# sepsamavi/safe-interactive-crowdnav

Hardware: AMD Instinct MI355X
Metric: sampled trajectories/sec (N x K, 50 denoise steps) (higher is better)
Workload: dtype fp16 activations x split-fp16 weights (weight-lo term as one bf8 MFMA per k64), fp32 accumulate; 1 GPU; cfg3: 256 episodes/GPU x N=5 x K=20 x H=12, 50 DDIM steps, JMID; episodes_per_gpu=256, total_episodes=256, humans=5, samples=20, horizon=12, denoise_steps=50, net=jmid, precision=f16mx, class_default_precision=f16mx, lanes=2

## Files before the change

### safe-interactive-crowdnav_amd/csrc/common.hpp

```cpp
#pragma once
#include <hip/hip_runtime.h>
#include <hip/hip_fp16.h>
#include <stdint.h>

#include <atomic>
#include <mutex>

namespace jmid {

typedef float f32x4 __attribute__((ext_vector_type(4)));
typedef float f32x16 __attribute__((ext_vector_type(16)));
typedef _Float16 f16x8 __attribute__((ext_vector_type(8)));
typedef _Float16 f16x4 __attribute__((ext_vector_type(4)));
typedef _Float16 f16x2 __attribute__((ext_vector_type(2)));

constexpr int kWave = 64;
constexpr int kPeMaxLen = 24;

struct HyperLayout {
    int g1, b1, g3, b3, g4, b4, go, bo, total;
};
__host__ __device__ inline HyperLayout make_hyper_layout(int d_model, int d_mid, int d_low) {
    HyperLayout L;
    L.g1 = 0;
// ... 55 lines not shown
    const Words w = __builtin_bit_cast(Words, a);
#pragma unroll
    for (unsigned i = 0; i < sizeof(T) / 4; ++i) asm volatile("" ::"s"(w.w[i]));
}
template <typename... T>
__device__ __forceinline__ void args_now_each(const T&... t) { (args_now(t), ...); }

__device__ __forceinline__ unsigned long long pin_uniform(unsigned long long v) {
    asm volatile("" : "+s"(v));
    return v;
}
__device__ __forceinline__ unsigned long long pin_uniform_rfl(unsigned long long v) {
    const unsigned lo = __builtin_amdgcn_readfirstlane((unsigned)v), hi = __builtin_amdgcn_readfirstlane((unsigned)(v >> 32));
    unsigned long long u = ((unsigned long long)hi << 32) | lo;
    asm volatile("" : "+s"(u));
    return u;
}

struct Tuning {
    int fuse_embed = 1;
    int ln_fuse = 0;
    int ln_rows = 0;
    int bystander_lds = 0;
    int gemm_h_variant = 0;
    int gemm_ng = 0;
    int no_vt_direct = 0;
    int attn_h_variant = 0;
    int attn_pack = 1;
    int vt_stage = 0;
    int graph = 0;
    int attn_nsplit = 0;
    int csl_swap = 0;
    int attn_sm = 0;
    int attn_prio = 0;
    int attn_one_wg = 0;
    int h1_stage = 0;
    int out_traj = 0;
    int attn_mx = 0;
    int mx_ln = 0;
    int attn_pf = 0;
    int gemm_small = 0;
    int small_cmb = 0;
    int small_lnx = 0;
    int cus = 256;
    int lnx_polls = 0;
    int lnx_withhold = 0;
    int small_lnx2 = 0;
    int gemm_pn = 0;
    int small_lanes = 0;
    int small_qk = 0;
    int small_pn = 0;
    int qkv0 = 0;
    int tail_fold = 0;
    int attn_abl = 0;
    int gemm_abl = 0;
};
#ifdef JMID_ABLATIONS
inline int attn_abl_bits(const Tuning& t) { return t.attn_abl; }
inline int gemm_abl_bits(const Tuning& t) { return t.gemm_abl; }
#else
inline int attn_abl_bits(const Tuning&) { return 0; }
inline int gemm_abl_bits(const Tuning&) { return 0; }
#endif

struct DevSeen {
    std::atomic<bool> v[64];
    DevSeen() { for (auto& b : v) b.store(false, std::memory_order_relaxed); }
};
struct DeviceOnce {
    std::unique_lock<std::mutex> lk;
    std::atomic<bool>* slot = nullptr;
    explicit operator bool() const { return slot != nullptr; }
    DeviceOnce() = default;
    DeviceOnce(DeviceOnce&& o) noexcept : lk(std::move(o.lk)), slot(o.slot) { o.slot = nullptr; }
    ~DeviceOnce() { if (slot) slot->store(true, std::memory_order_release); }
};
inline std::mutex& device_once_mutex() {
    static std::mutex m;
    return m;
}
inline DeviceOnce first_use_on_device(DevSeen& seen) {
    int dev = 0;
    (void)hipGetDevice(&dev);
    dev &= 63;
    DeviceOnce o;
    if (seen.v[dev].load(std::memory_order_acquire)) return o;
    o.lk = std::unique_lock<std::mutex>(device_once_mutex());
    if (seen.v[dev].load(std::memory_order_acquire)) {
        o.lk.unlock();
        return o;
    }
    o.slot = &seen.v[dev];
    return o;
}

template <auto Kernel, size_t MaxLds = 0, typename... Args>
inline hipError_t launch_with_lds(dim3 grid, dim3 block, size_t lds_bytes, hipStream_t st, Args... args) {
    static DevSeen seen;
    if (auto once_ = first_use_on_device(seen))
        (void)hipFuncSetAttribute(reinterpret_cast<const void*>(Kernel), hipFuncAttributeMaxDynamicSharedMemorySize,
                                  (int)(MaxLds ? MaxLds : lds_bytes));
    hipLaunchKernelGGL(Kernel, grid, block, lds_bytes, st, args...);
    return hipGetLastError();
}

template <typename F>
// ... 29 lines not shown
```

### safe-interactive-crowdnav_amd/csrc/gemm_f16x3.hpp

```cpp
#pragma once
#include <type_traits>
#include "common.hpp"
#include "gemm_f32.hpp"

namespace jmid {

typedef _Float16 half_t;
constexpr float kWScale = 256.0f;
constexpr float kWInv = 1.0f / 256.0f;
constexpr float kHalfMax = 60000.0f;

__device__ __forceinline__ void split_f32(float v, half_t& hi, half_t& lo) {
    asm("" : "+v"(v));
    hi = (half_t)v;
    lo = (half_t)(v - (float)hi);
}
__device__ __forceinline__ void split_f32_unscaled(float v, half_t& hi, half_t& lo) { split_f32(v, hi, lo); }
__device__ __forceinline__ unsigned char bf8_of_f16(half_t v) {
    return (unsigned char)((__builtin_bit_cast(unsigned short, v) + 0x80u) >> 8);
}

typedef int i32x2_s __attribute__((ext_vector_type(2)));
typedef unsigned short u16x2_s __attribute__((ext_vector_type(2)));
constexpr unsigned kHalfMaxBits = 0x7B53;
// ... 969 lines not shown
            __syncthreads();
            if (vt_staged_store<X2>(g, acc, m0 + wr * 64, n0 + wc * 128, lds + wid * 8192, l31, hi, lane)) return;
        }
    }
    gemm_h_epilogue<WM, WN, EPI, OUT, X2>(g, acc, m0, n0, wr, wc, l31, hi, BM, BN);
}

template <int EPI, int OUT, bool X2 = false>
inline hipError_t launch_gemm_h_dma256x256(const GemmHArgs& g, hipStream_t st, int flags = 3, int abl = 0) {
    const int ntm = (g.M + 255) / 256, ntn = g.N / 256;
    return launch_with_lds<&gemm_f16x3_dma256x256_kernel<EPI, OUT, X2>>(dim3(ntm * ntn), dim3(512), DMA3_LDS_BYTES, st, g, ntm, ntn,
                                                                         (abl & 8) ? 0 : 1, flags);
}

typedef int i32x4 __attribute__((ext_vector_type(4)));
typedef int i32x8 __attribute__((ext_vector_type(8)));

static __global__ void w8_image_kernel(const float* W, unsigned char* out, int N, int K, float scale) {
    const size_t n = (size_t)N * K;
    const int nb32 = N / 32;
    for (size_t i = (size_t)blockIdx.x * blockDim.x + threadIdx.x; i < n; i += (size_t)gridDim.x * blockDim.x) {
        const int r = (int)(i / K), k = (int)(i % K);
        float v = W[i] * scale;
        asm("" : "+v"(v));
        const half_t h = (half_t)v;
        const half_t lo = (half_t)(v - (float)h);
        const int kb = k >> 6, kk = k & 63, ksg = kk >> 4, hh = (kk >> 3) & 1, e = kk & 7;
        const int p = ksg * 8 + e, lane = (r & 31) + 32 * hh;
        const size_t o = ((((size_t)kb * nb32 + (r >> 5)) * 2 + (p >> 4)) * 64 + lane) * 16 + (p & 15);
        out[o] = (unsigned char)((__builtin_bit_cast(unsigned short, lo) + 0x80u) >> 8);
    }
}

__device__ __forceinline__ int bf8_of_f16x4(int d0, int d1) {
    return (int)__builtin_amdgcn_perm((unsigned)(d1 + 0x00800080), (unsigned)(d0 + 0x00800080), 0x07050301u);
}

template <int WR, int WC, int WM, int WN, int NS>
struct MxCfg {
    static constexpr int NT = 64 * WR * WC, BM = 32 * WM * WR, BN = 32 * WN * WC;
    static constexpr int A_HALFS = BM * 32, W_HALFS = BN * 32, STAGE = A_HALFS + W_HALFS;
    static constexpr int W8_BYTES = BN * 64;
    static constexpr int PIECE = NT * 8;
    static constexpr int NA = A_HALFS / PIECE, NW = W_HALFS / PIECE, N8 = W8_BYTES / (NT * 16);
    static constexpr size_t W8_OFF = size_t(NS) * STAGE * sizeof(half_t);
    static constexpr size_t RING_BYTES = W8_OFF + 2 * W8_BYTES;
    static constexpr size_t VT_BYTES = (WM == 2 && WN == 4) ? size_t(WR * WC) * 16384 : 0;
    static constexpr size_t LDS_BYTES = RING_BYTES > VT_BYTES ? RING_BYTES : VT_BYTES;
    static_assert(NA >= 1 && NW >= 1 && N8 >= 1 && A_HALFS % PIECE == 0 && W_HALFS % PIECE == 0, "tile / workgroup mismatch");
};
template <int N>
__device__ __forceinline__ void wait_vmcnt() { asm volatile("s_waitcnt vmcnt(%0)" ::"n"(N) : "memory"); }

template <int EPI, int OUT, int WR, int WC, int WM, int WN, int NS, bool K8IMG = false>
__global__ __launch_bounds__(64 * WR * WC, (WR * WC == 4 && WM == 2 && NS > 2) ? 1 : 2) void gemm_mx_kernel(GemmHArgs g, int ntm, int ntn, int stage_vt) {
    using C = MxCfg<WR, WC, WM, WN, NS>;
    constexpr int BM = C::BM, BN = C::BN, L = NS - 1;
    extern __shared__ __attribute__((aligned(16))) unsigned char lds_raw[];
    half_t* lds = reinterpret_cast<half_t*>(lds_raw);
    const int tid = threadIdx.x, lane = tid & 63, wid = tid >> 6;
    const int l31 = lane & 31, hi = lane >> 5;
    const int wr = wid / WC, wc = wid % WC;
    const int nwg = gridDim.x, b = blockIdx.x;
    const int q8 = nwg / 8, r8 = nwg % 8, xcd = b % 8;
    const int swz = (xcd < r8 ? xcd * (q8 + 1) : r8 * (q8 + 1) + (xcd - r8) * q8) + b / 8;
    const int gw = (stage_vt >> 8) ? (stage_vt >> 8) : ntn;
    const int per_g = ntm * gw, cg = swz / per_g, rem_g = swz - cg * per_g;
    const int tm = rem_g / gw, tn = cg * gw + (rem_g - tm * gw);
    const int m0 = tm * BM, n0 = tn * BN;
    const int nk = g.K / GEMMH_BK;
    const int nrb = (g.M + 127) / 128;
    const half_t* srcA[C::NA];
    const half_t* srcW[C::NW];
#pragma unroll
    for (int p = 0; p < C::NA; ++p) {
        const int h0 = (m0 & 127) * 32 + p * C::PIECE;
        int rb = m0 / 128 + h0 / 4096;
        rb = rb < nrb ? rb : nrb - 1;
        srcA[p] = g.Ahi + (size_t)rb * nk * 4096 + h0 % 4096;
    }
#pragma unroll
    for (int p = 0; p < C::NW; ++p) {
        const int h0 = (n0 & 127) * 32 + p * C::PIECE;
        srcW[p] = g.Whi + (size_t)(n0 / 128 + h0 / 4096) * nk * 4096 + h0 % 4096;
    }
    const unsigned char* src8 = g.W8 + (size_t)(n0 / 32) * 2048;
    unsigned lane_off = (unsigned)tid * 16u;
    const size_t w8_kstride = (size_t)(g.N / 32) * 2048;
    unsigned char* lds8 = lds_raw + C::W8_OFF;
    auto dma16 = [&](const void* s, void* d) {
        const unsigned long long u = pin_uniform(reinterpret_cast<unsigned long long>(s));
        __builtin_amdgcn_global_load_lds(reinterpret_cast<const __attribute__((address_space(1))) char*>(u) + lane_off,
                                         (__attribute__((address_space(3))) void*)d, 16, 0, 0);
    };
    const int wid_s = __builtin_amdgcn_readfirstlane(wid);
    auto issue = [&](int kt, int stg) {
        half_t* st = lds + stg * C::STAGE + wid_s * 512;
#pragma unroll
        for (int p = 0; p < C::NA; ++p) dma16(srcA[p] + (size_t)kt * 4096, st + p * C::PIECE);
#pragma unroll
        for (int p = 0; p < C::NW; ++p) dma16(srcW[p] + (size_t)kt * 4096, st + C::A_HALFS + p * C::PIECE);
        if (kt & 1) {
            const unsigned char* s8 = src8 + (size_t)(kt >> 1) * w8_kstride;
            unsigned char* d8 = lds8 + ((kt >> 1) & 1) * C::W8_BYTES + wid_s * 1024;
#pragma unroll
            for (int q = 0; q < C::N8; ++q) dma16(s8 + q * C::NT * 16, d8 + q * C::NT * 16);
        }
    };
    f32x16 acc[WM][WN];
#pragma unroll
    for (int i = 0; i < WM; ++i)
#pragma unroll
        for (int j = 0; j < WN; ++j)
#pragma unroll
            for (int r = 0; r < 16; ++r) acc[i][j][r] = 0.f;
    int offA[WM][2], offW[WN][2];
#pragma unroll
    for (int i = 0; i < WM; ++i) {
        const int row = wr * WM * 32 + i * 32 + l31, r = row & 127;
#pragma unroll
        for (int ks = 0; ks < 2; ++ks)
            offA[i][ks] = (row >> 7) * DMA_PLANE + r * 32 + (((ks * 2 + hi) ^ ((r >> 2) & 3)) * 8);
    }
#pragma unroll
    for (int j = 0; j < WN; ++j) {
        const int row = wc * WN * 32 + j * 32 + l31, r = row & 127;
#pragma unroll
        for (int ks = 0; ks < 2; ++ks)
            offW[j][ks] = C::A_HALFS + (row >> 7) * DMA_PLANE + r * 32 + (((ks * 2 + hi) ^ ((r >> 2) & 3)) * 8);
    }
    i32x8 a8[WM];
    auto tile = [&](const half_t* st, auto half_c, auto swap_c) {
        constexpr int HALF = decltype(half_c)::value;
        constexpr bool SWAP = decltype(swap_c)::value;
#pragma unroll
        for (int ks = 0; ks < 2; ++ks) {
            f16x8 ah[WM], wh[WN];
#pragma unroll
            for (int i = 0; i < WM; ++i) ah[i] = *reinterpret_cast<const f16x8*>(st + offA[i][ks]);
#pragma unroll
            for (int j = 0; j < WN; ++j) wh[j] = *reinterpret_cast<const f16x8*>(st + offW[j][ks]);
#pragma unroll
            for (int i = 0; i < WM; ++i)
#pragma unroll
                for (int j = 0; j < WN; ++j)
                    acc[i][j] = SWAP ? __builtin_amdgcn_mfma_f32_32x32x16_f16(wh[j], ah[i], acc[i][j], 0, 0, 0)
                                     : __builtin_amdgcn_mfma_f32_32x32x16_f16(ah[i], wh[j], acc[i][j], 0, 0, 0);
#pragma unroll
            for (int i = 0; i < WM; ++i) {
                const i32x4 d = __builtin_bit_cast(i32x4, ah[i]);
                a8[i][HALF * 4 + ks * 2 + 0] = bf8_of_f16x4(d[0], d[1]);
                a8[i][HALF * 4 + ks * 2 + 1] = bf8_of_f16x4(d[2], d[3]);
            }
        }
    };
    auto top = [&](int kt, int stg_next, auto par_c) {
        constexpr int P = decltype(par_c)::value;
        constexpr int n_odd = P == 0 ? L / 2 : (L - 1) / 2;
        if (kt + L - 1 < nk) wait_vmcnt<(L - 1) * (C::NA + C::NW) + n_odd * C::N8>();
        else wait_vmcnt<0>();
        __builtin_amdgcn_s_barrier();
        __builtin_amdgcn_sched_barrier(0);
        asm volatile("" : "+v"(lane_off));
        if (kt + L < nk) issue(kt + L, stg_next);
    };
    auto kloop = [&](auto swap_c) {
        constexpr bool SWAP = decltype(swap_c)::value;
#pragma unroll
        for (int t = 0; t < L; ++t)
            if (t < nk) issue(t, t);
        int stg = 0;
        for (int kt = 0; kt < nk; kt += 2) {
            const int s1 = stg + 1 == NS ? 0 : stg + 1, s2 = s1 + 1 == NS ? 0 : s1 + 1;
            top(kt, stg == 0 ? NS - 1 : stg - 1, std::integral_constant<int, 0>{});
            tile(lds + stg * C::STAGE, std::integral_constant<int, 0>{}, swap_c);
            __builtin_amdgcn_sched_barrier(0);
            top(kt + 1, stg, std::integral_constant<int, 1>{});
            tile(lds + s1 * C::STAGE, std::integral_constant<int, 1>{}, swap_c);
            {
                const unsigned char* wb = lds8 + ((kt >> 1) & 1) * C::W8_BYTES;
                i32x8 w8[WN];
#pragma unroll
                for (int j = 0; j < WN; ++j) {
                    const unsigned char* p = wb + (size_t)((wc * WN + j) * 2) * 1024 + lane * 16;
                    const i32x4 lo = *reinterpret_cast<const i32x4*>(p);
                    const i32x4 up = *reinterpret_cast<const i32x4*>(p + 1024);
                    w8[j] = i32x8{lo[0], lo[1], lo[2], lo[3], up[0], up[1], up[2], up[3]};
                }
#pragma unroll
                for (int i = 0; i < WM; ++i)
#pragma unroll
                    for (int j = 0; j < WN; ++j)
                        acc[i][j] = SWAP ? __builtin_amdgcn_mfma_scale_f32_32x32x64_f8f6f4(w8[j], a8[i], acc[i][j], 1, 1, 0, 0, 0, 0)
                                         : __builtin_amdgcn_mfma_scale_f32_32x32x64_f8f6f4(a8[i], w8[j], acc[i][j], 1, 1, 0, 0, 0, 0);
            }
            __builtin_amdgcn_sched_barrier(0);
            stg = s2;
        }
    };
    if constexpr (OUT == OUT_QKV && WM == 2 && WN == 4) {
        if (((stage_vt & 2) || (K8IMG && g.K8h && (n0 >= g.d || g.Q8l))) && n0 < 2 * g.d && g.d % 128 == 0) {
            kloop(std::true_type{});
            __syncthreads();
            qk_staged_store<K8IMG>(g, acc, m0 + wr * 64, n0 + wc * 128, lds + wid * 8192, l31, hi, lane);
            return;
        }
    }
    if constexpr ((EPI == EPI_CSL && (OUT == OUT_F32 || OUT == OUT_SPLIT)) || (EPI == EPI_BIAS_RELU && OUT == OUT_SPLIT)) {
        if (stage_vt & (EPI == EPI_CSL ? 4 : 8)) {
            kloop(std::true_type{});
            csl_swapped_epilogue<WM, WN, EPI, OUT, true>(g, acc, m0 + wr * WM * 32, n0 + wc * WN * 32, l31, hi);
            return;
        }
    }
    if constexpr (EPI == EPI_BIAS_RELU && OUT == OUT_SPLIT && WM == 2 && WN == 4) {
        if (stage_vt & 16) {
            kloop(std::true_type{});
            __syncthreads();
            h1_staged_store(g, acc, m0 + wr * 64, n0 + wc * 128, lds + wid * 8192, l31, hi, lane);
            return;
        }
    }
    kloop(std::false_type{});
    if constexpr (OUT == OUT_QKV && WM == 2 && WN == 4) {
        if (g.vt_direct && g.hd == 128 && n0 >= 2 * g.d && (stage_vt & 1)) {
            __syncthreads();
            if (vt_staged_store<true>(g, acc, m0 + wr * 64, n0 + wc * 128, lds + wid * 8192, l31, hi, lane)) return;
        }
    }
    gemm_h_epilogue<WM, WN, EPI, OUT, true, OUT == OUT_QKV && !(WM == 2 && WN == 4)>(g, acc, m0, n0, wr, wc, l31, hi, BM, BN);
}

template <int EPI, int OUT, int WR, int WC, int WM, int WN, int NS, bool K8IMG = false>
inline hipError_t launch_gemm_mx_cfg(const GemmHArgs& g, hipStream_t st, int flags, int group_tiles) {
    using C = MxCfg<WR, WC, WM, WN, NS>;
    if constexpr (OUT == OUT_QKV && WM == 2 && WN == 4 && !K8IMG)
        if (g.K8h) return launch_gemm_mx_cfg<EPI, OUT, WR, WC, WM, WN, NS, true>(g, st, flags, group_tiles);
    const int ntm = (g.M + C::BM - 1) / C::BM, ntn = g.N / C::BN;
    return launch_with_lds<&gemm_mx_kernel<EPI, OUT, WR, WC, WM, WN, NS, K8IMG>>(dim3(ntm * ntn), dim3(C::NT), C::LDS_BYTES, st, g, ntm, ntn,
                                                                                  flags | (group_tiles << 8));
}

constexpr int DMA64_PLANE = 64 * 32;
constexpr int DMA64_STAGE = 4 * DMA64_PLANE;
constexpr size_t DMA64_LDS_BYTES = size_t(4) * DMA64_STAGE * sizeof(half_t);

template <int EPI, int OUT, bool X2 = false>
__global__ __launch_bounds__(256, 2) void gemm_f16x3_dma64_kernel(GemmHArgs g, int ntm, int ntn) {
    constexpr int WM = 1, WN = 1, BM = 64, BN = 64;
    extern __shared__ __attribute__((aligned(16))) unsigned char lds_raw[];
    half_t* lds = reinterpret_cast<half_t*>(lds_raw);
    const int tid = threadIdx.x, lane = tid & 63, wid = tid >> 6;
    const int l31 = lane & 31, hi = lane >> 5;
    const int wr = wid >> 1, wc = wid & 1;
    const int nwg = gridDim.x, b = blockIdx.x;
    const int q8 = nwg / 8, r8 = nwg % 8, xcd = b % 8;
    const int swz = (xcd < r8 ? xcd * (q8 + 1) : r8 * (q8 + 1) + (xcd - r8) * q8) + b / 8;
    const int tm = swz / ntn, tn = swz - tm * ntn;
    const int m0 = tm * BM, n0 = tn * BN;
    const int nk = g.K / GEMMH_BK;
    const half_t* src[4];
    src[0] = g.Ahi + ((size_t)(tm >> 1) * nk) * 4096 + (tm & 1) * 2048 + tid * 8;
    src[1] = g.Alo + ((size_t)(tm >> 1) * nk) * 4096 + (tm & 1) * 2048 + tid * 8;
    src[2] = g.Whi + ((size_t)(tn >> 1) * nk) * 4096 + (tn & 1) * 2048 + tid * 8;
    src[3] = g.Wlo + ((size_t)(tn >> 1) * nk) * 4096 + (tn & 1) * 2048 + tid * 8;
    auto issue = [&](int kt) {
        half_t* st = lds + (kt & 3) * DMA64_STAGE + wid * 512;
#pragma unroll
        for (int i = 0; i < 4; ++i)
            __builtin_amdgcn_global_load_lds((const __attribute__((address_space(1))) void*)(src[i] + (size_t)kt * 4096),
                                             (__attribute__((address_space(3))) void*)(st + i * DMA64_PLANE), 16, 0, 0);
    };
    f32x16 accm[1][1];
#pragma unroll
    for (int r = 0; r < 16; ++r) {
        accm[0][0][r] = 0.f;
    }
    const int rowA = wr * 32 + l31, rowW = wc * 32 + l31;
    int offA[2], offW[2];
#pragma unroll
    for (int ks = 0; ks < 2; ++ks) {
        offA[ks] = rowA * 32 + (((ks * 2 + hi) ^ ((rowA >> 2) & 3)) * 8);
        offW[ks] = rowW * 32 + (((ks * 2 + hi) ^ ((rowW >> 2) & 3)) * 8);
    }
    issue(0);
    if (nk > 1) issue(1);
    if (nk > 2) issue(2);
    for (int kt = 0; kt < nk; ++kt) {
        if (kt + 2 < nk) asm volatile("s_waitcnt vmcnt(8)" ::: "memory");
        else if (kt + 1 < nk) asm volatile("s_waitcnt vmcnt(4)" ::: "memory");
        else asm volatile("s_waitcnt vmcnt(0)" ::: "memory");
        __builtin_amdgcn_s_barrier();
        __builtin_amdgcn_sched_barrier(0);
        if (kt + 3 < nk) issue(kt + 3);
        const half_t* st = lds + (kt & 3) * DMA64_STAGE;
#pragma unroll
        for (int ks = 0; ks < 2; ++ks) {
            f16x8 ah[1], al[1], wh[1], wl[1];
            ah[0] = *reinterpret_cast<const f16x8*>(st + offA[ks]);
            al[0] = *reinterpret_cast<const f16x8*>(st + DMA64_PLANE + offA[ks]);
            wh[0] = *reinterpret_cast<const f16x8*>(st + 2 * DMA64_PLANE + offW[ks]);
            wl[0] = *reinterpret_cast<const f16x8*>(st + 3 * DMA64_PLANE + offW[ks]);
            mfma3<1, 1, X2, csl_rowwise<EPI, OUT>()>(ah, al, wh, wl, accm);
        }
    }
    if constexpr (csl_rowwise<EPI, OUT>()) {
        csl_swapped_epilogue<WM, WN, EPI, OUT, X2>(g, accm, m0 + wr * WM * 32, n0 + wc * WN * 32, l31, hi);
        return;
    }
    gemm_h_epilogue<WM, WN, EPI, OUT, X2>(g, accm, m0, n0, wr, wc, l31, hi, BM, BN);
}

template <int EPI, int OUT, bool X2 = false>
inline hipError_t launch_gemm_h_dma64(const GemmHArgs& g, hipStream_t st) {
    const int ntm = (g.M + 63) / 64, ntn = (g.N + 63) / 64;
    return launch_with_lds<&gemm_f16x3_dma64_kernel<EPI, OUT, X2>>(dim3(ntm * ntn), dim3(256), DMA64_LDS_BYTES, st, g, ntm, ntn);
}

template <int EPI, int OUT, bool X2>
inline hipError_t launch_gemm_h_mode(const GemmHArgs& g, const GemmPlan& p, hipStream_t st) {
    switch (p.shape) {
        case GS_REG_64: return launch_gemm_h_cfg<1, 1, EPI, OUT, X2>(g, st);
        case GS_REG_128: return launch_gemm_h_cfg<2, 2, EPI, OUT, X2>(g, st);
        case GS_64: return launch_gemm_h_dma64<EPI, OUT, X2>(g, st);
        case GS_128: return launch_gemm_h_dma<EPI, OUT, X2>(g, st);
        case GS_256x128: return launch_gemm_h_dma256<EPI, OUT, X2>(g, st, p.group_tiles, p.abl);
        case GS_256x256:
            if constexpr (gemm_shape_built(GM_X2, EPI, OUT, GS_256x256)) return launch_gemm_h_dma256x256<EPI, OUT, X2>(g, st, p.flags, p.abl);
            return hipErrorInvalidValue;
        default: return hipErrorInvalidValue;
    }
}

template <int EPI, int OUT>
inline hipError_t launch_gemm_mx(const GemmHArgs& g, const GemmPlan& p, hipStream_t st) {
    switch (p.shape) {
        case GS_64: return launch_gemm_mx_cfg<EPI, OUT, 2, 2, 1, 1, 4>(g, st, p.flags, p.group_tiles);
        case GS_128: return launch_gemm_mx_cfg<EPI, OUT, 2, 2, 2, 2, 4>(g, st, p.flags, p.group_tiles);
        case GS_256x128:
            if constexpr (gemm_shape_built(GM_MX, EPI, OUT, GS_256x128)) return launch_gemm_mx_cfg<EPI, OUT, 4, 2, 2, 2, 3>(g, st, p.flags, p.group_tiles);
            return hipErrorInvalidValue;
        case GS_256x256:
            if constexpr (gemm_shape_built(GM_MX, EPI, OUT, GS_256x256)) return launch_gemm_mx_cfg<EPI, OUT, 4, 2, 2, 4, 2>(g, st, p.flags, p.group_tiles);
            return hipErrorInvalidValue;
#ifdef JMID_DIAGNOSTICS
        case GS_128x256:
            if constexpr (gemm_shape_built(GM_MX, EPI, OUT, GS_128x256)) return launch_gemm_mx_cfg<EPI, OUT, 2, 2, 2, 4, 2>(g, st, p.flags, p.group_tiles);
            return hipErrorInvalidValue;
        case GS_256x256_NS3:
            if constexpr (gemm_shape_built(GM_MX, EPI, OUT, GS_256x256_NS3)) return launch_gemm_mx_cfg<EPI, OUT, 4, 2, 2, 4, 3>(g, st, p.flags, p.group_tiles);
            return hipErrorInvalidValue;
#endif
        default: return hipErrorInvalidValue;
    }
}

template <int EPI, int OUT>
inline hipError_t launch_gemm_small(const GemmHArgs& g, const GemmPlan& p, hipStream_t st);

template <int EPI, int OUT>
inline hipError_t launch_gemm_h(const GemmHArgs& g, const GemmPlan& p, hipStream_t st) {
    if (gemm_shape_small(p.shape)) return launch_gemm_small<EPI, OUT>(g, p, st);
    if (p.mode == GM_MX) return launch_gemm_mx<EPI, OUT>(g, p, st);
    return p.mode == GM_X2 ? launch_gemm_h_mode<EPI, OUT, true>(g, p, st) : launch_gemm_h_mode<EPI, OUT, false>(g, p, st);
}

static __global__ void split_planes_kernel(const float* in, half_t* hi, half_t* lo, size_t n, int* range_flag) {
    bool overflow = false;
    for (size_t i = (size_t)blockIdx.x * blockDim.x + threadIdx.x; i < n; i += (size_t)gridDim.x * blockDim.x) {
        const float v = in[i];
        half_t h, l;
        split_f32(v, h, l);
        overflow |= !(fabsf(v) <= kHalfMax);
        hi[i] = h;
        lo[i] = l;
    }
    if (overflow && range_flag) atomicOr(range_flag, 1);
}

static __global__ void split_planes_blocked_kernel(const float* in, half_t* hi, half_t* lo, int rows, int K, int* range_flag,
                                            float scale) {
    bool overflow = false;
    const size_t n = (size_t)rows * K;
    for (size_t i = (size_t)blockIdx.x * blockDim.x + threadIdx.x; i < n; i += (size_t)gridDim.x * blockDim.x) {
        const int r = (int)(i / K), k = (int)(i % K);
        const float v = in[i] * scale;
        half_t h, l;
        split_f32(v, h, l);
        overflow |= !(fabsf(v) <= kHalfMax);
        const size_t o = blk_index(r, k, K);
        hi[o] = h;
        lo[o] = l;
    }
    if (overflow && range_flag) atomicOr(range_flag, 1);
}

// ... 63 lines not shown
```

### safe-interactive-crowdnav_amd/csrc/jmid_abi.hip

```cpp
#include "jmid_ctx.hpp"
#include "collision_stats.hpp"
#include "wall_stats.hpp"
#include "repair.hpp"

namespace jmid_host {

int upload_walls(jmid_ctx* h, int L, const double* walls, const double** dev, const std::string& who) {
    *dev = nullptr;
    if (L < 0 || L > WLS_MAX_L) return fail(h, JMID_EINVAL, who + " supports 0 <= L <= 64 walls");
    if (L == 0) return 0;
    if (!walls) return fail(h, JMID_EINVAL, who + ": null walls with L > 0");
    for (int i = 0; i < L * 4; ++i)
        if (!std::isfinite(walls[i])) return fail(h, JMID_EINVAL, who + ": a wall has a non-finite coordinate");
    if (int rc = h->wall_seg.upload(h, walls, L * 8, who.c_str())) return rc;
    *dev = h->wall_seg.get<double>();
    return 0;
}

std::string& thread_error() {
    static thread_local std::string e;
    return e;
}

int fail(jmid_ctx* h, int code, const std::string& msg) {
// ... 1683 lines not shown
}

int jmid_set_chunk_episodes(jmid_handle_t h, int episodes) {
    if (!h || episodes < 0) return JMID_EINVAL;
    h->chunk_eps = episodes;
    drop_graphs(h);
    return JMID_OK;
}

int jmid_set_tuning(jmid_handle_t h, const char* key, int value) {
    if (!h || !key) return JMID_EINVAL;
    const std::string k(key);
    struct Knob {
        const char* name;
        int Tuning::*field;
        int lo, hi;
    };
#ifdef JMID_DIAGNOSTICS
    static const Knob knobs[] = {
        {"gemm_h_variant", &Tuning::gemm_h_variant, 0, 8},
        {"attn_pack", &Tuning::attn_pack, 0, 1},
        {"fuse_embed", &Tuning::fuse_embed, 0, 1},
        {"bystander_lds", &Tuning::bystander_lds, 0, 160 * 1024},
        {"ln_rows", &Tuning::ln_rows, 0, 128},
        {"ln_fuse", &Tuning::ln_fuse, 0, 2},
        {"no_vt_direct", &Tuning::no_vt_direct, 0, 1},
        {"gemm_ng", &Tuning::gemm_ng, 0, 64},
        {"attn_h_variant", &Tuning::attn_h_variant, 0, 2},
        {"vt_stage", &Tuning::vt_stage, 0, 3},
        {"graph", &Tuning::graph, 0, 2},
        {"attn_nsplit", &Tuning::attn_nsplit, 0, 16},
        {"attn_mx", &Tuning::attn_mx, 0, 3},
        {"out_traj", &Tuning::out_traj, 0, 2},
        {"attn_pf", &Tuning::attn_pf, 0, 2},
        {"attn_one_wg", &Tuning::attn_one_wg, 0, 1},
        {"attn_sm", &Tuning::attn_sm, 0, 2},
        {"attn_prio", &Tuning::attn_prio, 0, 2},
        {"mx_ln", &Tuning::mx_ln, 0, 2},
        {"csl_swap", &Tuning::csl_swap, 0, 3},
        {"h1_stage", &Tuning::h1_stage, 0, 2},
        {"gemm_small", &Tuning::gemm_small, 0, 2},
        {"gemm_pn", &Tuning::gemm_pn, 0, 8},
        {"small_lanes", &Tuning::small_lanes, 0, 2},
        {"small_cmb", &Tuning::small_cmb, 0, 2},
        {"small_lnx", &Tuning::small_lnx, 0, 2},
        {"cus", &Tuning::cus, 0, 4096},
        {"lnx_polls", &Tuning::lnx_polls, 0, 1 << 20},
        {"lnx_withhold", &Tuning::lnx_withhold, 0, 1},
        {"small_lnx2", &Tuning::small_lnx2, 0, 2},
        {"small_qk", &Tuning::small_qk, 0, 2},
        {"small_pn", &Tuning::small_pn, 0, 8},
        {"qkv0", &Tuning::qkv0, 0, 2},
        {"tail_fold", &Tuning::tail_fold, 0, 2},
#ifdef JMID_ABLATIONS
        {"attn_abl", &Tuning::attn_abl, 0, 1 << 30},
        {"gemm_abl", &Tuning::gemm_abl, 0, 1 << 30},
#endif
    };
#endif
    if (k == "lanes") {
        if (value < 1 || value > jmid_ctx::kMaxLanes) return fail(h, JMID_EINVAL, "lanes must be 1..4");
        h->lanes = value;
        return JMID_OK;
    }
#ifdef JMID_DIAGNOSTICS
    for (const Knob& kn : knobs)
        if (k == kn.name) {
            if (value < kn.lo || value > kn.hi || (k == "ln_rows" && value != 0 && value != 64 && value != 128))
                return fail(h, JMID_EINVAL, k + " out of range");
            h->tune.*(kn.field) = value;
            if (k == "cus" && value == 0) {
                int cus = 0;
                h->tune.cus = hipDeviceGetAttribute(&cus, hipDeviceAttributeMultiprocessorCount, h->device) == hipSuccess && cus > 0 ? cus : 256;
            }
            drop_graphs(h);
            return JMID_OK;
        }
#endif
    return fail(h, JMID_EINVAL, "unknown tuning key " + k);
}

int64_t jmid_graph_replays(jmid_handle_t h) { return h ? h->graph_replays : -1; }

int64_t jmid_erange_count(jmid_handle_t h) { return h ? h->erange_calls : -1; }
int64_t jmid_timeout_count(jmid_handle_t h) { return h ? h->lnx_timeouts : -1; }

int jmid_set_caller_stream(jmid_handle_t h, void* stream) {
    if (!h) return JMID_EINVAL;
    h->caller_stream = reinterpret_cast<hipStream_t>(stream);
    return JMID_OK;
}

int jmid_synchronize(jmid_handle_t h) {
    if (!h) return JMID_EINVAL;
    HIPCHK(h, hipSetDevice(h->device));
    HIPCHK(h, hipStreamSynchronize(h->stream));
    return JMID_OK;
}

}
```

### safe-interactive-crowdnav_amd/csrc/launch_plan.hpp

```cpp
#pragma once
#include "common.hpp"

namespace jmid {

enum GemmEpi { EPI_BIAS = 0, EPI_BIAS_RELU = 1, EPI_CSL = 2 };
enum GemmOut { OUT_F32 = 0, OUT_SPLIT = 1, OUT_QKV = 2, OUT_LNX = 4 };

struct CallFacts {
    int small_now = 1;
    int one_chunk = 1;
    int attn_nsplit = 1;
    int qkv0_steps = 1;
    int tail_steps = 1;
};

enum GemmMode { GM_X3 = 0, GM_X2 = 1, GM_MX = 2 };

enum GemmShape {
    GS_NONE = 0,
    GS_SMALL_64x64, GS_SMALL_64x128, GS_SMALL_64x128_TWO,
    GS_SMALL_64x64_TWO,
    GS_64, GS_128, GS_256x128, GS_256x256,
    GS_128x256, GS_256x256_NS3,
    GS_REG_64, GS_REG_128,
};
constexpr int gemm_shape_bm(GemmShape s) {
    return s == GS_256x128 || s == GS_256x256 || s == GS_256x256_NS3 ? 256 : s == GS_128 || s == GS_128x256 || s == GS_REG_128 ? 128 : 64;
}
constexpr int gemm_shape_bn(GemmShape s) {
    return s == GS_256x256 || s == GS_128x256 || s == GS_256x256_NS3 ? 256
           : s == GS_SMALL_64x64 || s == GS_SMALL_64x64_TWO || s == GS_64 || s == GS_REG_64 ? 64 : 128;
}
constexpr bool gemm_shape_small(GemmShape s) { return s >= GS_SMALL_64x64 && s <= GS_SMALL_64x64_TWO; }

constexpr bool gemm_shape_built(GemmMode mode, int epi, int out, GemmShape s) {
    switch (s) {
        case GS_SMALL_64x64: return true;
        case GS_SMALL_64x128: return out != OUT_LNX;
        case GS_SMALL_64x128_TWO: return out != OUT_LNX && mode != GM_X3;
        case GS_SMALL_64x64_TWO: return out == OUT_LNX && mode == GM_MX;
        case GS_64:
        case GS_128: return out != OUT_LNX;
        case GS_256x128: return out != OUT_LNX && !(mode == GM_MX && epi == EPI_CSL && out == OUT_F32);
        case GS_256x256: return out != OUT_LNX && epi != EPI_CSL;
        case GS_128x256:
        case GS_256x256_NS3: return out != OUT_LNX && epi != EPI_CSL && mode == GM_MX;
        case GS_REG_64:
        case GS_REG_128: return out != OUT_LNX && mode != GM_MX;
        default: return false;
    }
}

struct GemmPlan {
    GemmMode mode;
    GemmShape shape;
    int flags, group_tiles, abl;
};

constexpr int kLnxMaxTiles = 64;

inline GemmShape small_gemm_shape(GemmMode mode, int out, int M, int N, int K, const CallFacts& cf, const Tuning& t) {
    if (t.gemm_small == 1 || t.gemm_h_variant != 0 || !cf.small_now || K % 128 != 0) return GS_NONE;
    const long ntm = (M + 63) / 64;
    if (out == OUT_LNX) {
        if (cf.small_now != 1 || cf.one_chunk != 1 || t.small_lnx == 2 || ntm > kLnxMaxTiles) return GS_NONE;
        if (ntm * 8 <= t.cus) return GS_SMALL_64x64;
        return gemm_shape_built(mode, 0, out, GS_SMALL_64x64_TWO) && ntm * 8 <= 2L * t.cus && t.small_lnx2 != 2 ? GS_SMALL_64x64_TWO : GS_NONE;
    }
    if (N % 128 != 0) return GS_NONE;
    const bool two = gemm_shape_built(mode, 0, out, GS_SMALL_64x128_TWO) && ntm * (N / 128) <= 512;
    if (cf.small_now == 2) return two ? GS_SMALL_64x128_TWO : GS_NONE;
    if (ntm * (N / 64) <= 256) return GS_SMALL_64x64;
    if (ntm * (N / 128) <= 256) return GS_SMALL_64x128;
    return two && t.gemm_small != 2 ? GS_SMALL_64x128_TWO : GS_NONE;
}

inline GemmShape large_gemm_shape(GemmMode mode, int epi, int out, int M, int N, const Tuning& t) {
    const auto usable = [&](GemmShape s) { return gemm_shape_built(mode, epi, out, s) && N % gemm_shape_bn(s) == 0; };
    constexpr GemmShape forced[9] = {GS_NONE, GS_REG_64, GS_REG_128, GS_128, GS_256x128, GS_64, GS_256x256, GS_128x256, GS_256x256_NS3};
    const GemmShape f = forced[t.gemm_h_variant >= 0 && t.gemm_h_variant <= 8 ? t.gemm_h_variant : 0];
    if (f != GS_NONE && gemm_shape_built(mode, epi, out, f) && (gemm_shape_bn(f) != 256 || N % 256 == 0)) return f;
    const long mt256 = (M + 255) / 256, big = (long)((M + 127) / 128) * ((N + 127) / 128);
    if (big < 256) return GS_64;
    const auto eff = [](long nb) { return (double)nb / (double)(((nb + 255) / 256) * 256); };
    const long nb256 = mt256 * ((N + 127) / 128);
    const int rows = mode == GM_MX ? 7168 : 12288;
    if (usable(GS_256x256)) {
        const long nbq = mt256 * (N / 256);
        if ((nbq >= 256 && 1.2 * eff(nbq) >= eff(nb256)) || (nbq < 256 && M >= rows)) return GS_256x256;
    }
    if (gemm_shape_built(mode, epi, out, GS_256x128) && nb256 >= 256 && 1.2 * eff(nb256) >= eff(big)) return GS_256x128;
    return GS_128;
}

inline int gemm_flags(const Tuning& t, bool small) {
    const int csl = (t.csl_swap == 2 ? 0 : 4) | (t.csl_swap == 3 ? 8 : 0);
    if (small) return csl | (t.small_qk == 2 ? 16 : 0);
    return (t.vt_stage == 2 ? 0 : (t.vt_stage == 3 ? 1 : 3)) | csl | (t.h1_stage == 2 ? 0 : 16);
}

inline int small_pick_groups(int M, int N, int K, int ntn, double w_bytes_per_el, double a_bytes_per_el) {
    const double wb = (double)N * K * w_bytes_per_el, ab = (double)M * K * a_bytes_per_el;
    int best = 1;
    double best_bytes = 8.0 * wb + ab;
    for (int pn = 2; pn <= 8; pn *= 2) {
        if (ntn % pn != 0) break;
        const double bytes = 8.0 * wb / pn + pn * ab;
        if (bytes < best_bytes) {
            best = pn;
            best_bytes = bytes;
        }
    }
    return best;
}

inline GemmPlan plan_gemm(GemmMode want, int epi, int out, int M, int N, int K, const CallFacts& cf, const Tuning& t) {
    GemmPlan p{};
    const bool mx_ok = K % 64 == 0 && N % 128 == 0 && t.gemm_h_variant != 1 && t.gemm_h_variant != 2;
    p.mode = want == GM_MX && !mx_ok ? GM_X2 : want;
    p.abl = gemm_abl_bits(t);
    p.shape = small_gemm_shape(p.mode, out, M, N, K, cf, t);
    const bool small = p.shape != GS_NONE;
    if (!small && out != OUT_LNX) p.shape = large_gemm_shape(p.mode, epi, out, M, N, t);
    if (p.shape == GS_NONE) return p;
    p.flags = small || p.mode == GM_MX ? gemm_flags(t, small) : p.shape == GS_256x256 ? gemm_flags(t, false) & 3 : 0;
    const int ntn = N / gemm_shape_bn(p.shape);
    if (small) {
        const int pn = t.small_pn > 0 ? (ntn % t.small_pn == 0 ? t.small_pn : 1)
                                      : small_pick_groups(M, N, K, ntn, p.mode == GM_MX ? 3.0 : 4.0, p.mode == GM_X3 ? 4.0 : 2.0);
        p.group_tiles = ntn / pn;
    } else if (p.mode == GM_MX) {
        p.group_tiles = t.gemm_pn > 1 && ntn % t.gemm_pn == 0 ? ntn / t.gemm_pn : 0;
    } else if (p.shape == GS_256x128) {
        p.group_tiles = t.gemm_ng;
    }
    return p;
}

inline int plan_ln_rows(bool second_generation, int M, const Tuning& t) {
    if (second_generation) return t.ln_rows == 64 ? 64 : 128;
    const auto fill = [](long n) { return (double)n / (double)(((n + 255) / 256) * 256); };
    const long n128 = (M + 127) / 128, n64 = (M + 63) / 64;
    return t.ln_rows == 128 || (t.ln_rows == 0 && 1.04 * fill(n128) >= fill(n64)) ? 128 : 64;
}

struct AttnPlan {
    bool dma;
    bool p1, pf;
    bool old_softmax;
    bool one_wg;
    int prio;
    int abl;
    int bystander_lds;
    bool pack;
    bool masked;
};
inline AttnPlan plan_attn(int head_dim, const Tuning& t) {
    AttnPlan p{};
    p.dma = head_dim == 128 && t.attn_h_variant != 1;
    p.p1 = t.attn_mx != 1;
    p.pf = t.attn_pf != 2;
    p.old_softmax = t.attn_sm == 2;
    p.one_wg = t.attn_one_wg != 0;
    p.prio = t.attn_prio;
    p.abl = attn_abl_bits(t);
    p.bystander_lds = t.bystander_lds;
    p.pack = t.attn_pack != 0;
    return p;
}

inline bool attn_masked_built(const AttnPlan& p, bool x2) { return !p.dma || (!p.old_softmax && !p.abl && (!x2 || (p.p1 && p.pf))); }

inline bool small_cmb_fits(const AttnPlan& ap, int nsplit, int x2, const Tuning& t) {
// ... 5 lines not shown
```

Measured before the change: 50980 traj/s.

## Add staggered wave-group K loop for the 256x256 MX GEMM

Adds a staggered K-loop variant for the 256x256 split-fp16 MX GEMM and makes it the default. Waves 4-7 run half a k-step behind waves 0-3 at raised priority, so that on each SIMD one wave's MFMAs overlap the other's LDS reads and barrier waits. The LDS layout becomes separate A and W rings with a three-stage depth, and each step waits for all outstanding loads (vmcnt 0) before a barrier. The old lockstep loop remains reachable only in diagnostics builds. The tail handling and the extra barriers could cost time on short K loops.

```diff
diff --git a/safe-interactive-crowdnav_amd/csrc/common.hpp b/safe-interactive-crowdnav_amd/csrc/common.hpp
--- a/safe-interactive-crowdnav_amd/csrc/common.hpp
+++ b/safe-interactive-crowdnav_amd/csrc/common.hpp
@@ -131,6 +131,7 @@
     int small_pn = 0;
     int qkv0 = 0;
     int tail_fold = 0;
+    int kloop_stagger = 0;
     int attn_abl = 0;
     int gemm_abl = 0;
 };
diff --git a/safe-interactive-crowdnav_amd/csrc/gemm_f16x3.hpp b/safe-interactive-crowdnav_amd/csrc/gemm_f16x3.hpp
--- a/safe-interactive-crowdnav_amd/csrc/gemm_f16x3.hpp
+++ b/safe-interactive-crowdnav_amd/csrc/gemm_f16x3.hpp
@@ -1045,10 +1045,13 @@
 template <int N>
 __device__ __forceinline__ void wait_vmcnt() { asm volatile("s_waitcnt vmcnt(%0)" ::"n"(N) : "memory"); }
 
-template <int EPI, int OUT, int WR, int WC, int WM, int WN, int NS, bool K8IMG = false>
+template <int EPI, int OUT, int WR, int WC, int WM, int WN, int NS, bool K8IMG = false, bool STAG = false>
 __global__ __launch_bounds__(64 * WR * WC, (WR * WC == 4 && WM == 2 && NS > 2) ? 1 : 2) void gemm_mx_kernel(GemmHArgs g, int ntm, int ntn, int stage_vt) {
     using C = MxCfg<WR, WC, WM, WN, NS>;
-    constexpr int BM = C::BM, BN = C::BN, L = NS - 1;
+    static_assert(!STAG || (WR * WC == 8 && NS == 3), "the staggered K loop: two waves per SIMD, a three-stage ring");
+    static_assert(!STAG || C::A_HALFS == C::W_HALFS, "the staggered K loop: one stage stride for both rings");
+    constexpr int BM = C::BM, BN = C::BN, L = STAG ? 1 : NS - 1;
+    constexpr int W_BASE = STAG ? NS * C::A_HALFS : C::A_HALFS, STRIDE = STAG ? C::A_HALFS : C::STAGE;
     extern __shared__ __attribute__((aligned(16))) unsigned char lds_raw[];
     half_t* lds = reinterpret_cast<half_t*>(lds_raw);
     const int tid = threadIdx.x, lane = tid & 63, wid = tid >> 6;
@@ -1081,13 +1084,13 @@
     unsigned lane_off = (unsigned)tid * 16u;
     const size_t w8_kstride = (size_t)(g.N / 32) * 2048;
     unsigned char* lds8 = lds_raw + C::W8_OFF;
-    auto dma16 = [&](const void* s, void* d) {
+    auto dma16 = [&](const void* s, void* d) __attribute__((always_inline)) {
         const unsigned long long u = pin_uniform(reinterpret_cast<unsigned long long>(s));
         __builtin_amdgcn_global_load_lds(reinterpret_cast<const __attribute__((address_space(1))) char*>(u) + lane_off,
                                          (__attribute__((address_space(3))) void*)d, 16, 0, 0);
     };
     const int wid_s = __builtin_amdgcn_readfirstlane(wid);
-    auto issue = [&](int kt, int stg) {
+    auto issue = [&](int kt, int stg) __attribute__((always_inline)) {
         half_t* st = lds + stg * C::STAGE + wid_s * 512;
 #pragma unroll
         for (int p = 0; p < C::NA; ++p) dma16(srcA[p] + (size_t)kt * 4096, st + p * C::PIECE);
@@ -1120,34 +1123,53 @@
         const int row = wc * WN * 32 + j * 32 + l31, r = row & 127;
 #pragma unroll
         for (int ks = 0; ks < 2; ++ks)
-            offW[j][ks] = C::A_HALFS + (row >> 7) * DMA_PLANE + r * 32 + (((ks * 2 + hi) ^ ((r >> 2) & 3)) * 8);
+            offW[j][ks] = W_BASE + (row >> 7) * DMA_PLANE + r * 32 + (((ks * 2 + hi) ^ ((r >> 2) & 3)) * 8);
     }
     i32x8 a8[WM];
-    auto tile = [&](const half_t* st, auto half_c, auto swap_c) {
-        constexpr int HALF = decltype(half_c)::value;
+    auto kstep = [&](const half_t* st, auto half_c, auto ks_c, auto swap_c) __attribute__((always_inline)) {
+        constexpr int HALF = decltype(half_c)::value, ks = decltype(ks_c)::value;
         constexpr bool SWAP = decltype(swap_c)::value;
-#pragma unroll
-        for (int ks = 0; ks < 2; ++ks) {
-            f16x8 ah[WM], wh[WN];
-#pragma unroll
-            for (int i = 0; i < WM; ++i) ah[i] = *reinterpret_cast<const f16x8*>(st + offA[i][ks]);
-#pragma unroll
-            for (int j = 0; j < WN; ++j) wh[j] = *reinterpret_cast<const f16x8*>(st + offW[j][ks]);
-#pragma unroll
-            for (int i = 0; i < WM; ++i)
-#pragma unroll
-                for (int j = 0; j < WN; ++j)
-                    acc[i][j] = SWAP ? __builtin_amdgcn_mfma_f32_32x32x16_f16(wh[j], ah[i], acc[i][j], 0, 0, 0)
-                                     : __builtin_amdgcn_mfma_f32_32x32x16_f16(ah[i], wh[j], acc[i][j], 0, 0, 0);
-#pragma unroll
-            for (int i = 0; i < WM; ++i) {
-                const i32x4 d = __builtin_bit_cast(i32x4, ah[i]);
-                a8[i][HALF * 4 + ks * 2 + 0] = bf8_of_f16x4(d[0], d[1]);
-                a8[i][HALF * 4 + ks * 2 + 1] = bf8_of_f16x4(d[2], d[3]);
-            }
-        }
-    };
-    auto top = [&](int kt, int stg_next, auto par_c) {
+        f16x8 ah[WM], wh[WN];
+#pragma unroll
+        for (int i = 0; i < WM; ++i) ah[i] = *reinterpret_cast<const f16x8*>(st + offA[i][ks]);
+#pragma unroll
+        for (int j = 0; j < WN; ++j) wh[j] = *reinterpret_cast<const f16x8*>(st + offW[j][ks]);
+#pragma unroll
+        for (int i = 0; i < WM; ++i)
+#pragma unroll
+            for (int j = 0; j < WN; ++j)
+                acc[i][j] = SWAP ? __builtin_amdgcn_mfma_f32_32x32x16_f16(wh[j], ah[i], acc[i][j], 0, 0, 0)
+                                 : __builtin_amdgcn_mfma_f32_32x32x16_f16(ah[i], wh[j], acc[i][j], 0, 0, 0);
+#pragma unroll
+        for (int i = 0; i < WM; ++i) {
+            const i32x4 d = __builtin_bit_cast(i32x4, ah[i]);
+            a8[i][HALF * 4 + ks * 2 + 0] = bf8_of_f16x4(d[0], d[1]);
+            a8[i][HALF * 4 + ks * 2 + 1] = bf8_of_f16x4(d[2], d[3]);
+        }
+    };
+    auto tile = [&](const half_t* st, auto half_c, auto swap_c) __attribute__((always_inline)) {
+        kstep(st, half_c, std::integral_constant<int, 0>{}, swap_c);
+        kstep(st, half_c, std::integral_constant<int, 1>{}, swap_c);
+    };
+    auto fp8_block = [&](int buf, auto swap_c) __attribute__((always_inline)) {
+        constexpr bool SWAP = decltype(swap_c)::value;
+        const unsigned char* wb = lds8 + buf * C::W8_BYTES;
+        i32x8 w8[WN];
+#pragma unroll
+        for (int j = 0; j < WN; ++j) {
+            const unsigned char* p = wb + (size_t)((wc * WN + j) * 2) * 1024 + lane * 16;
+            const i32x4 lo = *reinterpret_cast<const i32x4*>(p);
+            const i32x4 up = *reinterpret_cast<const i32x4*>(p + 1024);
+            w8[j] = i32x8{lo[0], lo[1], lo[2], lo[3], up[0], up[1], up[2], up[3]};
+        }
+#pragma unroll
+        for (int i = 0; i < WM; ++i)
+#pragma unroll
+            for (int j = 0; j < WN; ++j)
+                acc[i][j] = SWAP ? __builtin_amdgcn_mfma_scale_f32_32x32x64_f8f6f4(w8[j], a8[i], acc[i][j], 1, 1, 0, 0, 0, 0)
+                                 : __builtin_amdgcn_mfma_scale_f32_32x32x64_f8f6f4(a8[i], w8[j], acc[i][j], 1, 1, 0, 0, 0, 0);
+    };
+    auto top = [&](int kt, int stg_next, auto par_c) __attribute__((always_inline)) {
         constexpr int P = decltype(par_c)::value;
         constexpr int n_odd = P == 0 ? L / 2 : (L - 1) / 2;
         if (kt + L - 1 < nk) wait_vmcnt<(L - 1) * (C::NA + C::NW) + n_odd * C::N8>();
@@ -1157,8 +1179,7 @@
         asm volatile("" : "+v"(lane_off));
         if (kt + L < nk) issue(kt + L, stg_next);
     };
-    auto kloop = [&](auto swap_c) {
-        constexpr bool SWAP = decltype(swap_c)::value;
+    auto kloop_lockstep = [&](auto swap_c) __attribute__((always_inline)) {
 #pragma unroll
         for (int t = 0; t < L; ++t)
             if (t < nk) issue(t, t);
@@ -1170,26 +1191,82 @@
             __builtin_amdgcn_sched_barrier(0);
             top(kt + 1, stg, std::integral_constant<int, 1>{});
             tile(lds + s1 * C::STAGE, std::integral_constant<int, 1>{}, swap_c);
-            {
-                const unsigned char* wb = lds8 + ((kt >> 1) & 1) * C::W8_BYTES;
-                i32x8 w8[WN];
-#pragma unroll
-                for (int j = 0; j < WN; ++j) {
-                    const unsigned char* p = wb + (size_t)((wc * WN + j) * 2) * 1024 + lane * 16;
-                    const i32x4 lo = *reinterpret_cast<const i32x4*>(p);
-                    const i32x4 up = *reinterpret_cast<const i32x4*>(p + 1024);
-                    w8[j] = i32x8{lo[0], lo[1], lo[2], lo[3], up[0], up[1], up[2], up[3]};
-                }
-#pragma unroll
-                for (int i = 0; i < WM; ++i)
-#pragma unroll
-                    for (int j = 0; j < WN; ++j)
-                        acc[i][j] = SWAP ? __builtin_amdgcn_mfma_scale_f32_32x32x64_f8f6f4(w8[j], a8[i], acc[i][j], 1, 1, 0, 0, 0, 0)
-                                         : __builtin_amdgcn_mfma_scale_f32_32x32x64_f8f6f4(a8[i], w8[j], acc[i][j], 1, 1, 0, 0, 0, 0);
-            }
+            fp8_block((kt >> 1) & 1, swap_c);
             __builtin_amdgcn_sched_barrier(0);
             stg = s2;
         }
+    };
+    auto issue_s = [&](int kt, int stg_off, auto odd_c) __attribute__((always_inline)) {
+        half_t* st = lds + stg_off + wid_s * 512;
+#pragma unroll
+        for (int p = 0; p < C::NA; ++p) dma16(srcA[p] + (size_t)kt * 4096, st + p * C::PIECE);
+#pragma unroll
+        for (int p = 0; p < C::NW; ++p) dma16(srcW[p] + (size_t)kt * 4096, st + W_BASE + p * C::PIECE);
+        if constexpr (decltype(odd_c)::value) {
+            const unsigned char* s8 = src8 + (size_t)(kt >> 1) * w8_kstride;
+            unsigned char* d8 = lds8 + ((kt >> 1) & 1) * C::W8_BYTES + wid_s * 1024;
+#pragma unroll
+            for (int q = 0; q < C::N8; ++q) dma16(s8 + q * C::NT * 16, d8 + q * C::NT * 16);
+        }
+    };
+    auto rendezvous = [&]() __attribute__((always_inline)) {
+        wait_vmcnt<0>();
+        __builtin_amdgcn_s_barrier();
+        __builtin_amdgcn_sched_barrier(0);
+        asm volatile("" : "+v"(lane_off));
+    };
+    constexpr std::integral_constant<int, 0> c0{};
+    constexpr std::integral_constant<int, 1> c1{};
+    auto kloop_stagger = [&](auto swap_c) __attribute__((always_inline)) {
+        issue_s(0, 0, std::false_type{});
+        int s0 = 0, s1 = STRIDE, s2 = 2 * STRIDE;
+        if (wid_s < 4) {
+            for (int kt = 0; kt < nk; kt += 2) {
+                rendezvous();
+                issue_s(kt + 1, s1, std::true_type{});
+                tile(lds + s0, c0, swap_c);
+                __builtin_amdgcn_sched_barrier(0);
+                rendezvous();
+                if (kt + 2 < nk) issue_s(kt + 2, s2, std::false_type{});
+                tile(lds + s1, c1, swap_c);
+                fp8_block((kt >> 1) & 1, swap_c);
+                __builtin_amdgcn_sched_barrier(0);
+                const int t = s1;
+                s1 = s0; s0 = s2; s2 = t;
+            }
+        } else {
+            __builtin_amdgcn_s_setprio(1);
+            rendezvous();
+            issue_s(1, s1, std::true_type{});
+            kstep(lds + s0, c0, c0, swap_c);
+            __builtin_amdgcn_sched_barrier(0);
+            for (int kt = 0; kt + 2 < nk; kt += 2) {
+                rendezvous();
+                kstep(lds + s0, c0, c1, swap_c);
+                __builtin_amdgcn_sched_barrier(0);
+                issue_s(kt + 2, s2, std::false_type{});
+                kstep(lds + s1, c1, c0, swap_c);
+                __builtin_amdgcn_sched_barrier(0);
+                rendezvous();
+                kstep(lds + s1, c1, c1, swap_c);
+                fp8_block((kt >> 1) & 1, swap_c);
+                __builtin_amdgcn_sched_barrier(0);
+                issue_s(kt + 3, s0, std::true_type{});
+                kstep(lds + s2, c0, c0, swap_c);
+                __builtin_amdgcn_sched_barrier(0);
+                const int t = s1;
+                s1 = s0; s0 = s2; s2 = t;
+            }
+            rendezvous();
+            kstep(lds + s0, c0, c1, swap_c);
+            kstep(lds + s1, c1, c0, swap_c);
+            kstep(lds + s1, c1, c1, swap_c);
+            fp8_block(((nk >> 1) - 1) & 1, swap_c);
+        }
+    };
+    auto kloop = [&](auto swap_c) __attribute__((always_inline)) {
+        if constexpr (STAG) kloop_stagger(swap_c);
+        else kloop_lockstep(swap_c);
     };
     if constexpr (OUT == OUT_QKV && WM == 2 && WN == 4) {
         if (((stage_vt & 2) || (K8IMG && g.K8h && (n0 >= g.d || g.Q8l))) && n0 < 2 * g.d && g.d % 128 == 0) {
@@ -1224,13 +1301,13 @@
     gemm_h_epilogue<WM, WN, EPI, OUT, true, OUT == OUT_QKV && !(WM == 2 && WN == 4)>(g, acc, m0, n0, wr, wc, l31, hi, BM, BN);
 }
 
-template <int EPI, int OUT, int WR, int WC, int WM, int WN, int NS, bool K8IMG = false>
+template <int EPI, int OUT, int WR, int WC, int WM, int WN, int NS, bool K8IMG = false, bool STAG = false>
 inline hipError_t launch_gemm_mx_cfg(const GemmHArgs& g, hipStream_t st, int flags, int group_tiles) {
     using C = MxCfg<WR, WC, WM, WN, NS>;
     if constexpr (OUT == OUT_QKV && WM == 2 && WN == 4 && !K8IMG)
-        if (g.K8h) return launch_gemm_mx_cfg<EPI, OUT, WR, WC, WM, WN, NS, true>(g, st, flags, group_tiles);
+        if (g.K8h) return launch_gemm_mx_cfg<EPI, OUT, WR, WC, WM, WN, NS, true, STAG>(g, st, flags, group_tiles);
     const int ntm = (g.M + C::BM - 1) / C::BM, ntn = g.N / C::BN;
-    return launch_with_lds<&gemm_mx_kernel<EPI, OUT, WR, WC, WM, WN, NS, K8IMG>>(dim3(ntm * ntn), dim3(C::NT), C::LDS_BYTES, st, g, ntm, ntn,
+    return launch_with_lds<&gemm_mx_kernel<EPI, OUT, WR, WC, WM, WN, NS, K8IMG, STAG>>(dim3(ntm * ntn), dim3(C::NT), C::LDS_BYTES, st, g, ntm, ntn,
                                                                                   flags | (group_tiles << 8));
 }
 
@@ -1334,7 +1411,12 @@
             if constexpr (gemm_shape_built(GM_MX, EPI, OUT, GS_256x128)) return launch_gemm_mx_cfg<EPI, OUT, 4, 2, 2, 2, 3>(g, st, p.flags, p.group_tiles);
             return hipErrorInvalidValue;
         case GS_256x256:
-            if constexpr (gemm_shape_built(GM_MX, EPI, OUT, GS_256x256)) return launch_gemm_mx_cfg<EPI, OUT, 4, 2, 2, 4, 2>(g, st, p.flags, p.group_tiles);
+            if constexpr (gemm_shape_built(GM_MX, EPI, OUT, GS_256x256)) {
+#ifdef JMID_DIAGNOSTICS
+                if (p.lockstep) return launch_gemm_mx_cfg<EPI, OUT, 4, 2, 2, 4, 2>(g, st, p.flags, p.group_tiles);
+#endif
+                return launch_gemm_mx_cfg<EPI, OUT, 4, 2, 2, 4, 3, false, true>(g, st, p.flags, p.group_tiles);
+            }
             return hipErrorInvalidValue;
 #ifdef JMID_DIAGNOSTICS
         case GS_128x256:
diff --git a/safe-interactive-crowdnav_amd/csrc/jmid_abi.hip b/safe-interactive-crowdnav_amd/csrc/jmid_abi.hip
--- a/safe-interactive-crowdnav_amd/csrc/jmid_abi.hip
+++ b/safe-interactive-crowdnav_amd/csrc/jmid_abi.hip
@@ -1759,6 +1759,7 @@
         {"small_pn", &Tuning::small_pn, 0, 8},
         {"qkv0", &Tuning::qkv0, 0, 2},
         {"tail_fold", &Tuning::tail_fold, 0, 2},
+        {"kloop_stagger", &Tuning::kloop_stagger, 0, 2},
 #ifdef JMID_ABLATIONS
         {"attn_abl", &Tuning::attn_abl, 0, 1 << 30},
         {"gemm_abl", &Tuning::gemm_abl, 0, 1 << 30},
diff --git a/safe-interactive-crowdnav_amd/csrc/launch_plan.hpp b/safe-interactive-crowdnav_amd/csrc/launch_plan.hpp
--- a/safe-interactive-crowdnav_amd/csrc/launch_plan.hpp
+++ b/safe-interactive-crowdnav_amd/csrc/launch_plan.hpp
@@ -55,6 +55,7 @@
     GemmMode mode;
     GemmShape shape;
     int flags, group_tiles, abl;
+    int lockstep;
 };
 
 constexpr int kLnxMaxTiles = 64;
@@ -119,6 +120,7 @@
     const bool mx_ok = K % 64 == 0 && N % 128 == 0 && t.gemm_h_variant != 1 && t.gemm_h_variant != 2;
     p.mode = want == GM_MX && !mx_ok ? GM_X2 : want;
     p.abl = gemm_abl_bits(t);
+    p.lockstep = t.kloop_stagger == 2;
     p.shape = small_gemm_shape(p.mode, out, M, N, K, cf, t);
     const bool small = p.shape != GS_NONE;
     if (!small && out != OUT_LNX) p.shape = large_gemm_shape(p.mode, epi, out, M, N, t);
```

Measured after the change: 51390 traj/s, median of 6. About the same (+0.8%).
